# scomup/point-cloud-registration

Measured on AMD Instinct MI355X. Metric: M-correspondences/sec, plane calc_H_g_e2 on the B-01 stand-in (1.06 M pts), higher is better.
Workload: dtype f32; 1 GPU; plane_b01; kind=plane, target_points=1060000, scan_points_per_gpu=1060000, parallelism=scan-shard x1, devices_visible=1, scan_points_job=1060000, gauss_newton_iters_to_converge=5, correspondences_last_step=1060000

## Files before the change

### include/pcr.h

```cpp
#ifndef PCR_H
#define PCR_H

#include <stdint.h>

#ifdef __cplusplus
extern "C" {
#endif

#define PCR_API __attribute__((visibility("default")))

#define PCR_ABI_VERSION 5

typedef int pcr_status;
enum {
    PCR_OK = 0,
    PCR_ERR_INVALID = -1,
    PCR_ERR_HIP = -2,
    PCR_ERR_NO_TARGET = -3,
    PCR_ERR_COMM = -4,
    PCR_ERR_SINGULAR = -5,
    PCR_ERR_NOMEM = -6,
    PCR_ERR_UNSUPPORTED = -7
};

// ... 275 lines not shown
PCR_API pcr_status pcr_fgr_solo_max(pcr_context *ctx, int64_t *m_max);

#define PCR_COMPAT_M_MAX 32768
#define PCR_COMPAT_K_MAX 64
PCR_API pcr_status pcr_compat_bits(pcr_context *ctx, const float *src, const float *dst, int64_t m, double d,
                                   uint64_t *bits );
PCR_API pcr_status pcr_compat_degrees(pcr_context *ctx, const float *src, const float *dst, int64_t m, double d, int64_t *deg1 ,
                                      int64_t *deg2 );
PCR_API pcr_status pcr_compat_consensus(pcr_context *ctx, const float *src, const float *dst, int64_t m, double d, int n_seeds, int k,
                                        int64_t *deg1_or_null , int64_t *deg2_or_null , int32_t *seeds ,
                                        int32_t *members , int32_t *scores , int *n_seeds_out);

enum { PCR_K_LINEARIZE = 0, PCR_K_FINALIZE = 1, PCR_K_NN = 2, PCR_K_REDUCE = 3, PCR_K_ALLREDUCE = 4, PCR_K_CERTIFY = 5, PCR_K_COUNT = 6 };
PCR_API pcr_status pcr_profile_enable(pcr_context *ctx, int on);
PCR_API pcr_status pcr_profile_reset(pcr_context *ctx);
PCR_API pcr_status pcr_profile_read(pcr_context *ctx, int64_t launches[PCR_K_COUNT], double total_ms[PCR_K_COUNT]);
PCR_API pcr_status pcr_profile_read_n(pcr_context *ctx, int capacity, int64_t *launches, double *total_ms, int *count);
PCR_API pcr_status pcr_target_index_info(pcr_target *t, double *cell, int64_t dims[3], int64_t *occupied, int64_t *n);
PCR_API pcr_status pcr_target_index_population(pcr_target *t, int64_t *pop_max, int64_t *pop_p99, int *heavy);
PCR_API pcr_status pcr_target_index_x_order(pcr_target *t, double *xq);
PCR_API int pcr_x_order_rule(int f32_point_target, int heavy, int64_t n, int cell_bits);
PCR_API pcr_status pcr_target_index_halo(pcr_target *t, double *halo, int64_t *records);
PCR_API pcr_status pcr_target_index_halo2(pcr_target *t, double *halo, int64_t *records);
PCR_API pcr_status pcr_target_filter_band(pcr_target *t, double *band);
PCR_API pcr_status pcr_nn_counters(pcr_target *t, pcr_scan *s, const double T[16], double max_dist, double out[11]);
PCR_API pcr_status pcr_nn_counters_x(pcr_target *t, pcr_scan *s, const double T[16], double max_dist, double out[3]);
PCR_API pcr_status pcr_nn_counters_edge(pcr_target *t, pcr_scan *s, const double T[16], double max_dist, double out[9]);
PCR_API pcr_status pcr_set_variant(pcr_context *ctx, int variant);
PCR_API pcr_status pcr_get_variant(pcr_context *ctx, int *variant);
PCR_API pcr_status pcr_set_nn_mode(pcr_context *ctx, int mode);
PCR_API pcr_status pcr_set_reuse(pcr_context *ctx, int mode, double tau, double mu);
PCR_API pcr_status pcr_get_reuse(pcr_context *ctx, int *mode, double *tau, double *mu);
PCR_API pcr_status pcr_scan_reuse_stats(pcr_scan *s, double out[8]);
PCR_API pcr_status pcr_context_host_fold_passes(pcr_context *ctx, uint64_t *passes);
PCR_API pcr_status pcr_set_fuse_finalize(pcr_context *ctx, int on);
PCR_API int pcr_has_dev_kernels(void);
PCR_API pcr_status pcr_get_pipeline(pcr_context *ctx, int *variant, int *fuse_finalize, int *nn_mode);

#ifdef __cplusplus
}
#endif
#endif
```

### point_cloud_registration_amd/_capi.py

```python

import atexit
import ctypes as C
import os
import weakref

import numpy as np

_HERE = os.path.dirname(os.path.abspath(__file__))
LIB_PATH = os.environ.get("PCR_LIB") or os.path.join(_HERE, "libpcr_hip.so")
DEV_LIB_PATH = os.path.join(_HERE, "libpcr_hip_dev.so")

PCR_OK = 0
PCR_ERR_INVALID, PCR_ERR_HIP, PCR_ERR_NO_TARGET, PCR_ERR_COMM, PCR_ERR_SINGULAR, PCR_ERR_NOMEM = -1, -2, -3, -4, -5, -6
PCR_ERR_UNSUPPORTED = -7
ICP, PLANE, VPLANE, NDT = 0, 1, 2, 3
FLAG_ICP_RR_QUIRK = 1
FLAG_NO_SCAN_SORT = 2
FLAG_LOCAL_ONLY = 4
FLAG_HOST_LOOP = 8
FLAG_DEVICE_LOOP = 16
FLAG_KEEP_ORDER = 32
K_LINEARIZE, K_FINALIZE, K_NN, K_REDUCE, K_ALLREDUCE, K_CERTIFY, K_COUNT = 0, 1, 2, 3, 4, 5, 6
KERNEL_NAMES = ("linearize", "finalize", "nn", "reduce", "allreduce", "certify")
NN_FULL, NN_TRACK, NN_LIST = 0, 1, 2
# ... 80 lines not shown
    "pcr_profile_enable": (C.c_int, [_vp, C.c_int]),
    "pcr_profile_reset": (C.c_int, [_vp]),
    "pcr_profile_read": (C.c_int, [_vp, _i64p, _f64p]),
    "pcr_target_index_info": (C.c_int, [_vp, C.POINTER(C.c_double), _i64p, C.POINTER(C.c_int64), C.POINTER(C.c_int64)]),
    "pcr_target_index_halo": (C.c_int, [_vp, C.POINTER(C.c_double), C.POINTER(C.c_int64)]),
    "pcr_target_index_population": (C.c_int, [_vp, C.POINTER(C.c_int64), C.POINTER(C.c_int64), C.POINTER(C.c_int)]),
    "pcr_target_index_x_order": (C.c_int, [_vp, C.POINTER(C.c_double)]),
    "pcr_x_order_rule": (C.c_int, [C.c_int, C.c_int, C.c_int64, C.c_int]),
    "pcr_set_variant": (C.c_int, [_vp, C.c_int]),
    "pcr_get_variant": (C.c_int, [_vp, C.POINTER(C.c_int)]),
    "pcr_set_nn_mode": (C.c_int, [_vp, C.c_int]),
    "pcr_set_fuse_finalize": (C.c_int, [_vp, C.c_int]),
    "pcr_get_pipeline": (C.c_int, [_vp, C.POINTER(C.c_int), C.POINTER(C.c_int), C.POINTER(C.c_int)]),
    "pcr_nn_counters": (C.c_int, [_vp, _vp, _f64p, C.c_double, _f64p]),
    "pcr_nn_counters_x": (C.c_int, [_vp, _vp, _f64p, C.c_double, _f64p]),
    "pcr_nn_counters_edge": (C.c_int, [_vp, _vp, _f64p, C.c_double, _f64p]),
    "pcr_set_reuse": (C.c_int, [_vp, C.c_int, C.c_double, C.c_double]),
    "pcr_get_reuse": (C.c_int, [_vp, C.POINTER(C.c_int), C.POINTER(C.c_double), C.POINTER(C.c_double)]),
    "pcr_scan_reuse_stats": (C.c_int, [_vp, _f64p]),
    "pcr_context_host_fold_passes": (C.c_int, [_vp, C.POINTER(C.c_uint64)]),
    "pcr_hash64": (C.c_int, [_vp, C.c_uint64, C.POINTER(C.c_uint64)]),
    "pcr_target_filter_band": (C.c_int, [_vp, C.POINTER(C.c_double)]),
    "pcr_target_index_halo2": (C.c_int, [_vp, C.POINTER(C.c_double), C.POINTER(C.c_int64)]),
    "pcr_usable_cpus": (C.c_int, []),
    "pcr_has_dev_kernels": (C.c_int, []),
    "pcr_abi_version": (C.c_int, []),
    "pcr_context_trim": (C.c_int, [_vp, C.POINTER(C.c_uint64)]),
    "pcr_profile_read_n": (C.c_int, [_vp, C.c_int, _i64p, _f64p, C.POINTER(C.c_int)]),
    "pcr_scan_read_matches": (C.c_int, [_vp, _vp]),
    "pcr_comm_p2p_finegrained": (C.c_int, [_vp, C.POINTER(C.c_int)]),
    "pcr_lzf_decompress": (C.c_int, [_vp, C.c_uint64, _vp, C.c_uint64, C.POINTER(C.c_uint64)]),
    "pcr_lzf_compress": (C.c_int, [_vp, C.c_uint64, _vp, C.c_uint64, C.POINTER(C.c_uint64)]),
    "pcr_gn_set": (C.c_int, [_vp, _vp, C.c_int, _vp, C.c_int, C.c_int64, C.c_int, _f64p]),
    "pcr_coreset": (C.c_int, [_vp, _f64p, C.c_int, C.c_int64, _f64p, C.c_int, C.c_int64, C.POINTER(C.c_int64), _f64p, _i64p,
                              _f64p]),
    "pcr_linearize_rows": (C.c_int, [_vp, _vp, C.c_int, _f64p, C.c_double, C.c_uint, _vp, _vp, _vp, _vp, _vp]),
    "pcr_linearize_weighted": (C.c_int, [_vp, _vp, C.c_int, _f64p, C.c_double, C.c_uint, _f64p, _f64p]),
    "pcr_scan_coreset": (C.c_int, [_vp, _vp, C.c_int, _f64p, C.c_double, C.c_uint, C.c_int, C.c_int64, _i64p, _f64p,
                                   C.POINTER(C.c_int64)]),
    "pcr_target_estimate_covariances": (C.c_int, [_vp, C.c_int, C.c_int, C.c_double, _vp]),
    "pcr_target_set_covariances": (C.c_int, [_vp, _f32p]),
    "pcr_target_get_covariances": (C.c_int, [_vp, _f32p]),
    "pcr_scan_estimate_covariances": (C.c_int, [_vp, C.c_int, C.c_int, C.c_double, _vp]),
    "pcr_scan_set_covariances": (C.c_int, [_vp, _f32p]),
    "pcr_scan_get_covariances": (C.c_int, [_vp, _f32p]),
    "pcr_gicp_linearize": (C.c_int, [_vp, _vp, _f64p, C.c_double, C.c_uint, _f64p]),
# ... 508 lines not shown
        out = np.empty((self.size(), 6), np.float64)
        check(lib().pcr_target_voxels_get_covariances(self.handle, out))
        return out

    def voxel_stats(self, names=("mean", "cov", "norm", "icov", "counts", "keys")):
        n = self.size()
        bufs = {"mean": np.empty((n, 3)), "cov": np.empty((n, 3, 3)), "norm": np.empty((n, 3)),
                "icov": np.empty((n, 3, 3)), "counts": np.empty(n, np.int64), "keys": np.empty(n, np.int64)}
        nv = C.c_int64(0)
        args = [_ptr(bufs[k]) if k in names else None for k in ("mean", "cov", "norm", "icov", "counts", "keys")]
        check(lib().pcr_target_voxels_get(self.handle, C.byref(nv), *args))
        return {k: bufs[k] for k in names}

    def index_info(self):
        cell, occ, n = C.c_double(0), C.c_int64(0), C.c_int64(0)
        dims = np.zeros(3, np.int64)
        check(lib().pcr_target_index_info(self.handle, C.byref(cell), dims, C.byref(occ), C.byref(n)))
        halo, nh = C.c_double(0), C.c_int64(0)
        check(lib().pcr_target_index_halo(self.handle, C.byref(halo), C.byref(nh)))
        band = C.c_double(0)
        check(lib().pcr_target_filter_band(self.handle, C.byref(band)))
        halo2, nh2 = C.c_double(0), C.c_int64(0)
        check(lib().pcr_target_index_halo2(self.handle, C.byref(halo2), C.byref(nh2)))
        pmax, p99, heavy = C.c_int64(0), C.c_int64(0), C.c_int(0)
        check(lib().pcr_target_index_population(self.handle, C.byref(pmax), C.byref(p99), C.byref(heavy)))
        xq = C.c_double(0)
        check(lib().pcr_target_index_x_order(self.handle, C.byref(xq)))
        return {"cell": cell.value, "dims": tuple(int(d) for d in dims), "occupied": occ.value, "n": n.value,
                "halo": halo.value, "halo_records": nh.value, "filter_band": band.value,
                "halo2": halo2.value, "halo2_records": nh2.value,
                "pop_max": pmax.value, "pop_p99": p99.value, "heavy": bool(heavy.value),
                "x_ordered": xq.value > 0.0, "xq": xq.value}

    def searches_f64(self):
        return bool(self.is_voxel or getattr(self, "has_f64", False))

    def nn_query(self, q, r_max=np.inf):
        q = np.asarray(q)
        if q.dtype == np.float64 and self.searches_f64():
            q = np.ascontiguousarray(q)
            m = q.shape[0]
            dist, idx = np.empty(m, np.float64), np.empty(m, np.int64)
            check(lib().pcr_nn_query_dd(self.handle, q, m, float(r_max), dist, idx))
            return dist, idx
        q = np.ascontiguousarray(q, dtype=np.float32)
        m = q.shape[0]
        idx = np.empty(m, np.int64)
        if self.searches_f64():
            dist = np.empty(m, np.float64)
            check(lib().pcr_nn_query_f64(self.handle, q, m, float(r_max), dist, idx))
        else:
            dist = np.empty(m, np.float32)
            check(lib().pcr_nn_query(self.handle, q, m, float(r_max), dist, idx))
# ... 907 lines not shown
```

### point_cloud_registration_amd/csrc/api.hip

```cpp
#include <math.h>
#include <stdarg.h>
#include <stdlib.h>
#include <string.h>

#include <string>

#include "gn_math.h"
#include "pcr_internal.h"

static thread_local std::string g_last_error;

void pcr_set_error(const char *fmt, ...) {
    char buf[1024];
    va_list ap;
    va_start(ap, fmt);
    vsnprintf(buf, sizeof buf, fmt, ap);
    va_end(ap);
    g_last_error = buf;
}

extern "C" const char *pcr_last_error(void) { return g_last_error.c_str(); }
extern "C" const char *pcr_version(void) { return "pcr-hip 0.4 (gfx950)"; }
extern "C" int pcr_abi_version(void) { return PCR_ABI_VERSION; }

// ... 407 lines not shown
extern "C" pcr_status pcr_profile_read(pcr_context *ctx, int64_t launches[PCR_K_COUNT], double total_ms[PCR_K_COUNT]) {
    return pcr_profile_read_n(ctx, PCR_K_COUNT, launches, total_ms, nullptr);
}

template <typename T>
static pcr_status upload(pcr_context *ctx, const T *host, size_t count, DevBuf<T> *buf, bool exact = false, bool sync = true) {
    HIP_TRY(exact ? buf->alloc_exact(count) : buf->alloc(count));
    if (count) {
        HIP_TRY(hipMemcpyAsync(buf->p, host, sizeof(T) * count, hipMemcpyHostToDevice, ctx->stream));
        if (sync) HIP_TRY(hipStreamSynchronize(ctx->stream));
    }
    return PCR_OK;
}
static pcr_status synced(pcr_context *ctx, pcr_status s) {
    if (s != PCR_OK) (void)hipStreamSynchronize(ctx->stream);
    return s;
}

void pcr_target_release(pcr_target *t);
static void target_free(pcr_target *t) { pcr_target_release(t); }
void pcr_target_release(pcr_target *t) {
    if (!t) return;
    target_free(t->filter);
    void *ptrs[] = {t->cell_start, t->cell_seed, t->rowocc, t->lbox, t->gbox, t->lbox_h, t->gbox_h, t->lbox_h2, t->gbox_h2, t->cs_h, t->pts_h, t->j_h, t->cs_h2, t->pts_h2, t->j_h2, t->pts, t->pn, t->col, t->cint, t->gcov, t->pts64, t->means, t->vnorm, t->vicov, t->vcov,
                    t->st_mean, t->st_cov, t->st_norm, t->st_icov, t->st_counts, t->st_keys};
    if (t->ctx) (void)hipSetDevice(t->ctx->device);
    for (void *p : ptrs) pcr_persist_free(t->ctx, p);
    delete t;
}

static pcr_status points_create_common(pcr_context *ctx, const float *d_xyz, int64_t n, const float *d_normals,
                                       float cell_hint, pcr_target **out) {
    pcr_target *t = new pcr_target();
    t->ctx = ctx; t->is_voxel = 0; t->n = n; t->serial = ctx->next_serial++;
    pcr_status s = pcr_build_point_grid(ctx, d_xyz, n, cell_hint, t);
    if (s == PCR_OK && d_normals) {
        hipError_t e = pcr_persist_alloc((void **)&t->pn, sizeof(PtN) * (size_t)(n ? n : 1));
        if (e != hipSuccess) { pcr_set_error("hipMalloc normals: %s", hipGetErrorString(e)); s = PCR_ERR_HIP; }
        else s = pcr_permute_normals(ctx, d_normals, n, t->pts, t->pn);
        if (s == PCR_OK && hipStreamSynchronize(ctx->stream) != hipSuccess) s = PCR_ERR_HIP;
    }
    if (s != PCR_OK) { target_free(t); return s; }
    *out = t;
    return PCR_OK;
}

extern "C" pcr_status pcr_target_points_create(pcr_context *ctx, const float *xyz, int64_t n,
                                               const float *normals_or_null, float cell_hint, pcr_target **out) {
    PCR_REQUIRE(ctx && out, "NULL argument");
    PCR_REQUIRE(n >= 0 && (xyz || n == 0), "bad point array");
// ... 153 lines not shown
extern "C" pcr_status pcr_target_index_population(pcr_target *t, int64_t *pop_max, int64_t *pop_p99, int *heavy) {
    PCR_REQUIRE(t, "NULL argument");
    if (pop_max || pop_p99) {
        HIP_TRY(hipSetDevice(t->ctx->device));
        CtxScope scope(t->ctx);
        PCR_TRY(pcr_cell_population(t->ctx, t));
    }
    if (pop_max) *pop_max = t->pop_max;
    if (pop_p99) *pop_p99 = t->pop_p99;
    if (heavy) *heavy = t->heavy ? 1 : 0;
    return PCR_OK;
}

extern "C" pcr_status pcr_target_index_halo(pcr_target *t, double *halo, int64_t *records) {
    PCR_REQUIRE(t, "NULL argument");
    const pcr_target *p = t->is_voxel ? t->filter : t;
    if (halo) *halo = p ? (double)p->gf.halo : 0.0;
    if (records) *records = p ? p->n_h : 0;
    return PCR_OK;
}

extern "C" pcr_status pcr_target_index_halo2(pcr_target *t, double *halo, int64_t *records) {
    PCR_REQUIRE(t, "NULL argument");
    if (halo) *halo = t->is_voxel ? 0.0 : (double)t->halo2;
    if (records) *records = t->is_voxel ? 0 : t->n_h2;
    return PCR_OK;
}

extern "C" pcr_status pcr_target_filter_band(pcr_target *t, double *band) {
    PCR_REQUIRE(t && band, "NULL argument");
    *band = (t->is_voxel && t->filter) ? t->filter_band : 0.0;
    return PCR_OK;
}

extern "C" pcr_status pcr_target_destroy(pcr_target *t) {
    if (!t) return PCR_OK;
    (void)hipSetDevice(t->ctx->device);
    (void)hipStreamSynchronize(t->ctx->stream);
    target_free(t);
    return PCR_OK;
}

extern "C" pcr_status pcr_scan_create_device(pcr_context *ctx, const float *d_xyz, int64_t n, unsigned flags,
                                             pcr_scan **out) {
    PCR_REQUIRE(ctx && out, "NULL argument");
    PCR_REQUIRE(n >= 0 && (d_xyz || n == 0), "bad scan array");
    CtxScope scope(ctx);
    pcr_scan *s = new pcr_scan();
// ... 277 lines not shown
```

### point_cloud_registration_amd/csrc/index_build.hip

```cpp
#include <hipcub/hipcub.hpp>
#include <rocprim/rocprim.hpp>

#include <math.h>
#include <cmath>
#include <vector>

#include "nn_device.h"
#include "gn_math.h"

__device__ __forceinline__ unsigned f2ord(float f) {
    const unsigned u = __float_as_uint(f);
    return (u & 0x80000000u) ? ~u : (u | 0x80000000u);
}
static inline float ord2f(unsigned u) {
    const unsigned v = (u & 0x80000000u) ? (u & 0x7fffffffu) : ~u;
    float f;
    memcpy(&f, &v, 4);
    return f;
}

#define BBOX_SLOTS 64
#define BBOX_STRIDE 32
#define BBOX_WORDS (BBOX_STRIDE * (1 + BBOX_SLOTS))
template <typename T>
// ... 817 lines not shown
    const char *env = use_env ? getenv("PCR_GRID_CELL") : nullptr;
    bool auto_h = !(cell_hint > 0);
    if (env && atof(env) > 0) { h = atof(env); auto_h = false; }
    double halo = n <= ((int64_t)1 << 24) ? halo_default : 0.0;
    const char *he = getenv("PCR_HALO");
    if (he && *he) halo = atof(he);
    bool heavy = false;
    PCR_TRY((build_grid<float, float, PtF>(ctx, d_xyz, n, h, auto_h, &t->gf, &t->cell_start, &t->cell_seed, &t->pts, &t->occupied,
                                           halo, &t->cs_h, &t->pts_h, &t->j_h, &t->n_h, use_env ? &heavy : nullptr)));
    t->heavy = heavy;
    if (heavy) {
        PCR_TRY(make_leaf_boxes(ctx, t->pts, n, t->gf.h, t->gf.slack, &t->lbox, &t->gbox));
        t->gf.lbox = t->lbox; t->gf.gbox = t->gbox;
        if (t->pts_h) {
            PCR_TRY(make_leaf_boxes(ctx, t->pts_h, t->n_h, t->gf.h, t->gf.slack, &t->lbox_h, &t->gbox_h));
            t->gf.lbox_h = t->lbox_h; t->gf.gbox_h = t->gbox_h;
        }
        HIP_TRY(hipStreamSynchronize(ctx->stream));
    }
    return PCR_OK;
}

pcr_status pcr_build_deep_lists(pcr_context *ctx, pcr_target *t) {
    if (t->is_voxel || !t->cs_h || t->n <= 0 || t->cs_h2) return PCR_OK;
    {
        const char *de = getenv("PCR_DEEP_LISTS");
        if (de && atoi(de) == 0) return PCR_OK;
        size_t free_b = 0, total_b = 0;
        if (hipMemGetInfo(&free_b, &total_b) != hipSuccess) { (void)hipGetLastError(); free_b = 0; }
        const char *mb = getenv("PCR_DEEP_LISTS_MB");
        const double budget = mb && *mb ? atof(mb) * 1048576.0 : (double)free_b / 16.0;
        const double grow = (1.0 + 2.0 * PCR_HALO2_FRAC) * (1.0 + 2.0 * PCR_HALO2_FRAC) / (1.2 * 1.2);
        const double est = (double)(t->n_h > 0 ? t->n_h : t->n) * grow * 20.0 + 4.0 * ((double)t->gf.nx * t->gf.ny * t->gf.nz);
        if (est > budget) return PCR_OK;
    }
    DevBuf<uint32_t> cs_h, j_h;
    DevBuf<PtF> pts_h;
    int64_t n_h = 0;
    PCR_TRY(build_halo_lists(ctx, t->gf, t->pts, t->n, t->cell_start, PCR_HALO2_FRAC, &cs_h, &pts_h, &j_h, &n_h));
    if (n_h <= 0) return PCR_OK;
    t->halo2 = (float)(PCR_HALO2_FRAC * (double)t->gf.h);
    t->n_h2 = n_h;
    t->cs_h2 = cs_h.release(); t->pts_h2 = pts_h.release(); t->j_h2 = j_h.release();
    if (t->heavy) {
        PCR_TRY(make_leaf_boxes(ctx, t->pts_h2, n_h, t->gf.h, t->gf.slack, &t->lbox_h2, &t->gbox_h2));
        HIP_TRY(hipStreamSynchronize(ctx->stream));
    }
    return PCR_OK;
}

pcr_status pcr_build_centroid_grid(pcr_context *ctx, const double *d_mean, int64_t n, double cell, pcr_target *t) {
    uint32_t *cs_h = nullptr, *j_h = nullptr; PtF *pts_h = nullptr; int64_t n_h = 0;
    PCR_TRY((build_grid<double, double, PtD>(ctx, d_mean, n, cell, false, &t->gd, &t->cell_start, &t->cell_seed, &t->means, &t->occupied,
                                             0.0, &cs_h, &pts_h, &j_h, &n_h)));
    const char *oe = getenv("PCR_ROW_OCC");
    if (n > 0 && !(oe && atoi(oe) == 0)) PCR_TRY(make_row_occ<double>(ctx, t->cell_start, &t->gd, &t->rowocc));
    return PCR_OK;
}

__global__ void __launch_bounds__(256) k_means_to_f32(const PtD *__restrict__ means, int64_t n, float *__restrict__ xyz) {
    const int64_t j = (int64_t)blockIdx.x * 256 + threadIdx.x;
    if (j >= n) return;
    const PtD m = means[j];
    xyz[3 * j] = (float)m.x; xyz[3 * j + 1] = (float)m.y; xyz[3 * j + 2] = (float)m.z;
}

pcr_status pcr_build_centroid_filter(pcr_context *ctx, pcr_target *t) {
    if (t->n <= 0 || !ctx->vox_filter) return PCR_OK;
    const Geom<double> &g = t->gd;
// ... 211 lines not shown
```

### point_cloud_registration_amd/csrc/kernels.hip

```cpp
#include <type_traits>

#include "pass_device.h"
#ifdef PCR_DEV
#include "nn_mfma.h"
#endif

template <int VOXEL>
__global__ void __launch_bounds__(256) k_certify(const LinArgs a) {
    PoseK P;
    PoseQ Q;
    if (!load_pose<false>(a, P)) return;
    load_prev(a, Q);
    const TileIter it(a);
    const int lane = threadIdx.x & 63;
    uint32_t marked = 0;
    for (int64_t i0 = it.base - threadIdx.x; i0 < it.end; i0 += it.stride) {
        const int64_t i = i0 + threadIdx.x;
        const bool live = i < it.end;
        bool cert = false;
        if (live) {
            const uint32_t j = a.nn_j[i];
            const float lb = a.lb2[i];
            const float x = a.sx[i], y = a.sy[i], z = a.sz[i];
            float tx, ty, tz, ux, uy, uz;
// ... 151 lines not shown
__global__ void __launch_bounds__(256) k_nn_fix(const LinArgs a) {
    PoseK P;
    if (!load_pose<false>(a, P)) return;
    if (__builtin_amdgcn_readfirstlane(*(volatile const uint32_t *)a.pending) != a.stamp) return;
    for (int64_t i = (int64_t)blockIdx.x * 256 + threadIdx.x; i < a.n; i += (int64_t)gridDim.x * 256) {
        const uint32_t j = a.nn_j[i];
        if (nn_is_pending(j)) nn_point_fix(a, P, i, j & ~PCR_PENDING_BIT);
    }
}
#endif

__device__ __forceinline__ void pose_write(PoseDev *p, const double *T) {
    for (int i = 0; i < 16; ++i) p->T[i] = T[i];
    for (int i = 0; i < 3; ++i) {
        for (int j = 0; j < 3; ++j) { p->R[3 * i + j] = T[4 * i + j]; p->r32[3 * i + j] = (float)T[4 * i + j]; }
        p->t32[i] = (float)T[4 * i + 3];
    }
}
__device__ __forceinline__ void pose_arm(PoseDev *p, const double *T, int max_iter) {
    pose_write(p, T);
    p->iter = 0;
    p->done = max_iter > 0 ? PCR_LOOP_RUNNING : PCR_LOOP_MAXITER;
    p->tile_local = 0;
    p->halo_deep = 1;
}

__device__ __forceinline__ void gn_update(const FinArgs &f, double (*A)[7]) {
    PoseDev *p = f.pose;
    const int it = p->iter;
    double T[16];
    for (int i = 0; i < 16; ++i) T[i] = p->T[i];
    if (f.trace) {
        double *row = f.trace + (size_t)it * 45;
        for (int i = 0; i < 16; ++i) row[i] = T[i];
        for (int i = 0; i < 29; ++i) row[16 + i] = f.out[i];
    }
    double T_old[16];
    for (int i = 0; i < 16; ++i) T_old[i] = T[i];
    const int r = gn_step(A, f.out, f.tol, T);
    const double moved = r == 0 ? gn_typical_motion(T_old, T, f.bb_c, f.bb_e) : 0.0;
    p->tile_local = (r == 0 && f.local_len > 0.0 && moved < f.local_len) ? 1 : 0;
    p->halo_deep = (r == 0 && moved >= f.deep_len) ? 1 : 0;
    int done = r == 2 ? PCR_LOOP_SINGULAR : (r == 1 ? PCR_LOOP_CONVERGED : PCR_LOOP_RUNNING);
    if (r == 0) pose_write(p, T);
    const int it1 = it + 1;
    if (done == PCR_LOOP_RUNNING && it1 >= f.max_iter) done = PCR_LOOP_MAXITER;
    p->iter = it1;
    p->done = done;
    if (f.host_T) {
        if (done != PCR_LOOP_RUNNING) {
            for (int i = 0; i < 16; ++i) f.host_T[i] = T[i];
            __threadfence_system();
        }
        *f.host_state = ((unsigned long long)(unsigned)done << 32) | (unsigned)it1;
    }
}

__global__ void __launch_bounds__(64) k_gn_update(const FinArgs f) {
    if (threadIdx.x != 0) return;
    if (f.pose->done == PCR_LOOP_RUNNING) {
        double A[6][7];
        gn_update(f, A);
    } else if (f.pose->done == PCR_LOOP_COMMFAIL && f.host_state) {
        *f.host_state = ((unsigned long long)(unsigned)PCR_LOOP_COMMFAIL << 32) | (unsigned)f.pose->iter;
    }
// ... 331 lines not shown
```

### point_cloud_registration_amd/csrc/pass.hip

```cpp
#include <stdlib.h>

#include "pass_device.h"

static int grid8(int64_t want, int64_t cap = INT64_MAX) {
    int64_t nb = (want + 7) & ~(int64_t)7;
    if (nb > (cap & ~(int64_t)7)) nb = cap & ~(int64_t)7;
    return nb < 8 ? 8 : (int)nb;
}

#define PCR_HOST_ROWS_BYTES (sizeof(double) * 8 * 32 + sizeof(uint32_t) * 8 * PCR_GFLAG_STRIDE)

static double cell_edge(const pcr_target *t) { return t->is_voxel ? t->gd.h : (double)t->gf.h; }

pcr_status pcr_ensure_scratch(pcr_context *ctx, int64_t n_points) {
    (void)n_points;
    if (!ctx->d_partials) {
        ctx->max_blocks = (ctx->num_cu * 16 + 7) & ~7;
        HIP_TRY(pcr_malloc_retry((void **)&ctx->d_partials, sizeof(double) * 32 * (size_t)(ctx->max_blocks + 8)));
        HIP_TRY(pcr_malloc_retry((void **)&ctx->d_out, sizeof(double) * 32));
        HIP_TRY(pcr_malloc_retry((void **)&ctx->d_pose, sizeof(PoseDev)));
        HIP_TRY(hipHostMalloc(&ctx->h_out, sizeof(double) * 64, hipHostMallocMapped | hipHostMallocCoherent));
        memset(ctx->h_out, 0, sizeof(double) * 64);
        HIP_TRY(hipHostGetDevicePointer((void **)&ctx->h_out_dev, ctx->h_out, 0));
        HIP_TRY(hipHostMalloc((void **)&ctx->h_rows, PCR_HOST_ROWS_BYTES, hipHostMallocMapped | hipHostMallocCoherent));
// ... 12 lines not shown
        ctx->nn_blocks_per_cu[1] = blocks_per_cu(PCR_OCC_VOXEL, 4);
        ctx->nn_blocks_per_cu[3] = blocks_per_cu(PCR_OCC_FILTER, 4);
    }
    return PCR_OK;
}

static int64_t blocks_wanted(const pcr_context *ctx, int64_t n) {
    const int64_t want = (n + 255) / 256, cap = (int64_t)ctx->num_cu * 8;
    return want < cap ? want : cap;
}
int choose_blocks(const pcr_context *ctx, int64_t n) { return grid8(blocks_wanted(ctx, n), ctx->max_blocks); }

struct Pass {
    pcr_context *ctx;
    pcr_target *t;
    pcr_scan *s;
    int kind;
    LinArgs a;
    FinArgs f;
    bool one_kernel;
    bool fused_fin;
    bool gn_inline;
    double motion;
    int nn_mode;
    bool reuse_ready;
    bool q6;
};

bool pcr_pass_is_fused(const pcr_context *ctx, const pcr_scan *s) {
    if (ctx->variant == 2) return s->n <= (int64_t)ctx->num_cu * 1024;
    return ctx->variant == 0;
}

static void set_filter_bound(LinArgs &a, double bound);
#define PCR_PUBLIC_FLAGS (PCR_FLAG_ICP_RR_QUIRK | PCR_FLAG_NO_SCAN_SORT | PCR_FLAG_LOCAL_ONLY | PCR_FLAG_HOST_LOOP | PCR_FLAG_DEVICE_LOOP | PCR_FLAG_KEEP_ORDER)

static bool pass_is_q6(const pcr_target *t, int kind) { return kind == PCR_PLANE && !t->is_voxel && t->pts64 != nullptr; }

static pcr_status refuse_comm_and_q6(const pcr_target *t, int kind, const char *passes, const char *plane_passes, const char *q6_note) {
    if (t->ctx->comm != nullptr) pcr_set_error("%s are not available on a context with a communicator attached (pcr_comm_*, pcr_group)", passes);
    else if (pass_is_q6(t, kind)) pcr_set_error("%s are not available over a float64 point target (%s)", plane_passes, q6_note);
    else return PCR_OK;
    return PCR_ERR_UNSUPPORTED;
}

static void pass_init(Pass *ps, pcr_target *t, pcr_scan *s, int kind, bool one_kernel, bool q6) {
// ... 79 lines not shown
    if (pcr_build_deep_lists(ctx, t) != PCR_OK) (void)hipGetLastError();
}

static void pass_fill_lin(Pass *ps, double max_dist, unsigned flags, bool use_filter, bool deep, int nblocks) {
    const pcr_context *ctx = ps->ctx;
    const pcr_target *t = ps->t;
    const pcr_scan *s = ps->s;
    LinArgs &a = ps->a;
    memset(&a, 0, sizeof a);
    a.sx = s->x; a.sy = s->y; a.sz = s->z; a.n = s->n;
    a.gf = t->gf; a.pts = t->pts; a.pn = t->pn;
    a.pts_last = (uint32_t)(t->is_voxel ? 0 : t->n + PCR_PTS_PAD - 1);
    a.gd = t->gd; a.means = t->means; a.vnorm = t->vnorm; a.vicov = t->vicov;
    a.cell_start = t->cell_start;
    if (use_filter) {
        a.gf = t->filter->gf; a.pts = t->filter->pts; a.cs_f = t->filter->cell_start;
        a.band_f = (float)(t->filter_band * 1.000001);
    }
    if (ps->q6) {
        a.gd = t->gq; a.means = t->pts64; a.cs_f = t->cell_start;
        a.band_f = (float)(t->band64 * 1.000001);
        flags |= PCR_IFLAG_NOGATE;
    }
    if (deep && t->cs_h2) { a.cs_h2 = t->cs_h2; a.pts_h2 = t->pts_h2; a.j_h2 = t->j_h2; a.halo2_f = t->halo2; a.lbox_h2 = t->lbox_h2; a.gbox_h2 = t->gbox_h2; }
    a.md_f = (float)max_dist; a.md_d = max_dist;
    const double bound = max_dist * (1.0 + 1e-6);
    a.bound2_f = (float)(bound * bound); a.bound2_d = bound * bound;
    set_filter_bound(a, bound);
    a.flags = flags;
    a.nblocks = nblocks;
    a.partials = ctx->d_partials;
    a.nn_j = s->nn_j; a.tile_ctr = ctx->d_tile_ctr + 9 * PCR_TICKET_STRIDE;
    a.pending = ctx->d_tile_ctr + 9 * PCR_TICKET_STRIDE + (size_t)PCR_TILE_CTRS * PCR_TILE_STRIDE;
    a.lb2 = s->lb2; a.umask = s->umask; a.ucnt = s->ucnt;
    a.mu_f = (float)(ctx->reuse_mu * cell_edge(t));
}

static void pass_fill_fin(Pass *ps) {
    const pcr_context *ctx = ps->ctx;
    const pcr_scan *s = ps->s;
    FinArgs &f = ps->f;
    memset(&f, 0, sizeof f);
    for (int i = 0; i < 3; ++i) { f.bb_c[i] = s->bb_c[i]; f.bb_e[i] = s->bb_e[i]; }
    f.local_len = ctx->local_frac * cell_edge(ps->t);
    f.deep_len = PCR_HALO2_MOVE * cell_edge(ps->t);
    f.ucnt = s->ucnt; f.n_ucnt = ps->a.nblocks;
    f.partials = ctx->d_partials; f.tile_ctr = ctx->d_tile_ctr + 9 * PCR_TICKET_STRIDE; f.tickets = ctx->d_tile_ctr;
    f.nblocks = ps->a.nblocks; f.kind = ps->kind; f.out = ctx->d_out;
}

static pcr_status pass_setup(Pass *ps, pcr_target *t, pcr_scan *s, int kind, double max_dist, unsigned flags, bool force_fused = false) {
    pcr_context *ctx = t->ctx;
    PCR_TRY(pass_validate(t, s, kind, max_dist));
    HIP_TRY(hipSetDevice(ctx->device));
    PCR_TRY(pcr_ensure_scratch(ctx, s->n));
    const bool q6 = pass_is_q6(t, kind);
    const bool one_kernel = (force_fused || pcr_pass_is_fused(ctx, s)) && !q6;
    pass_init(ps, t, s, kind, one_kernel, q6);
    const int nblocks_split = grid8(choose_blocks(ctx, s->n), ctx->num_cu * 4);
    PCR_TRY(pass_scan_buffers(ps, nblocks_split));
    const bool filter_ok = t->is_voxel && ctx->vox_filter && ctx->nn_mode != 3 && (!one_kernel || ctx->fuse_finalize);
    if (filter_ok) pass_lazy_filter(ctx, t, one_kernel);
    const bool deep_ok = !t->is_voxel && !one_kernel && !q6 && t->cs_h && nn_plain(ctx);
    if (deep_ok) pass_lazy_deep_lists(ctx, t);
    pass_fill_lin(ps, max_dist, flags & PCR_PUBLIC_FLAGS, filter_ok && t->filter, deep_ok, one_kernel ? choose_blocks(ctx, s->n) : nblocks_split);
    pass_fill_fin(ps);
    return PCR_OK;
}
// ... 112 lines not shown
            else if (a.pose != nullptr) local = mode == PCR_NN_FULL ? 2 : 0;
            else if (ps->motion >= 0.0 && ps->motion < ps->f.local_len) local = 1;
        }
        if (ctx->tile_local >= 0) local = ctx->tile_local;
        ps->a.sched_local = local;
#ifdef PCR_DEV
        const bool mfma = !vox && !ps->q6 && mode == PCR_NN_FULL && ps->t->n > 0 && ctx->nn_mode == 4;
        if (coop) {
            pcr_dev_launch_coop(nn_grid, ctx->stream, a);
        } else if (mfma) {
            const int64_t nbm = (int64_t)ctx->num_cu * ctx->nn_blocks_per_cu[4];
            launch_nn_mfma(ps->t->cs_h != nullptr, ps->a.sched_local == 1 ? 1 : 0, dim3((unsigned)grid8(nbm < g.need ? nbm : g.need)), ctx->stream, a);
        } else
#endif
        if (filter) {
            if (++ctx->filter_stamp == 0) {
                HIP_TRY(hipMemsetAsync(a.pending, 0, 4, ctx->stream));
                ctx->filter_stamp = 1;
            }
            ps->a.stamp = ctx->filter_stamp;
            const bool fhalo = ps->q6 ? ps->t->cs_h != nullptr : ps->t->filter->cs_h != nullptr;
            launch_nn_filter(fhalo, ps->a.sched_local == 1 ? 1 : 0, !ps->fused_fin, ps->q6, nn_grid, ctx->stream, a);
        } else {
            if (!vox && a.pose == nullptr && a.halo2_f > 0.f && mode == PCR_NN_FULL && !(ps->motion >= 0.0 && ps->motion < ps->f.deep_len)) {
                ps->a.gf.halo = a.halo2_f; ps->a.gf.cs_h = a.cs_h2; ps->a.gf.pts_h = a.pts_h2; ps->a.gf.j_h = a.j_h2;
                ps->a.gf.lbox_h = a.lbox_h2; ps->a.gf.gbox_h = a.gbox_h2;
            }
            launch_plain_search(ps, nn_grid);
        }
        ps->s->nn_serial = ps->t->serial;
    }
    pcr_prof_end(ctx, &ev);
    return PCR_OK;
}

static void enqueue_reduce(Pass *ps, dim3 grid, bool filter) {
    pcr_context *ctx = ps->ctx;
    ProfEvent ev;
    pcr_prof_begin(ctx, PCR_K_REDUCE, &ev);
    RoctxRange range("pcr:reduce");
#ifdef PCR_DEV
    if (!ps->fused_fin) pcr_dev_launch_reduce(ps->kind, grid, ctx->stream, ps->a);
    else
#endif
    launch_reduce_kind(ps->kind, filter, grid, ctx->stream, ps->a, ps->f);
    pcr_prof_end(ctx, &ev);
}

static pcr_status pass_enqueue(Pass *ps) {
// ... 505 lines not shown
```

### point_cloud_registration_amd/csrc/pass_device.h

```cpp
#pragma once

#include <string.h>
#include <time.h>

#include <type_traits>

#include "gn_math.h"
#include "nn_device.h"

struct PoseK {
    float r32[9], t32[3];
    double R[9];
};
struct PoseQ {
    float r32[9], t32[3];
};

struct LinArgs {
    const float *sx, *sy, *sz;
    int64_t n;
    Geom<float> gf;
    const PtF *pts;
    uint32_t pts_last;
    const PtN *pn;
// ... 5 lines not shown
    PoseK hp;
    const PoseDev *pose;
    PoseQ hq;
    float *lb2;
    unsigned long long *umask;
    uint32_t *ucnt;
    float mu_f;
    float md_f;
    double md_d;
    float bound2_f;
    double bound2_d;
    const uint32_t *cs_f;
    float band_f;
    float mu_ff;
    float bound2_ff;
    uint32_t *pending;
    uint32_t stamp;
    unsigned flags;
    int nblocks;
    double *partials;
    uint32_t *nn_j;
    uint32_t *tile_ctr;
    int sched_local;
    const uint32_t *cs_h2;
    const void *pts_h2;
    const uint32_t *j_h2;
    float halo2_f;
    const float4 *lbox_h2, *gbox_h2;
};

struct RowArgs {
    const uint32_t *order;
    double *J, *r, *w, *W;
    int64_t *idx;
    uint32_t *flag, *inv;
    const uint32_t *off;
    double *P;
    int64_t stride;
    int64_t *col_idx;
};

__device__ __forceinline__ Geom<float> select_lists(const LinArgs &a) {
    Geom<float> g = a.gf;
    if (a.pose != nullptr && a.halo2_f > 0.f && __builtin_amdgcn_readfirstlane(a.pose->halo_deep) != 0) {
        g.halo = a.halo2_f; g.cs_h = a.cs_h2; g.pts_h = a.pts_h2; g.j_h = a.j_h2; g.lbox_h = a.lbox_h2; g.gbox_h = a.gbox_h2;
    }
    return g;
}

__device__ __forceinline__ float uniform_f32(float v) { return __int_as_float(__builtin_amdgcn_readfirstlane(__float_as_int(v))); }
__device__ __forceinline__ double uniform_f64(double v) {
    return __hiloint2double(__builtin_amdgcn_readfirstlane(__double2hiint(v)), __builtin_amdgcn_readfirstlane(__double2loint(v)));
}

template <bool NEED_R>
__device__ __forceinline__ bool load_pose(const LinArgs &a, PoseK &P) {
    if (a.pose == nullptr) { P = a.hp; return true; }
    const PoseDev *p = a.pose;
    if (__builtin_amdgcn_readfirstlane(p->done) != 0) return false;
#pragma unroll
    for (int i = 0; i < 9; ++i) P.r32[i] = uniform_f32(p->r32[i]);
#pragma unroll
    for (int i = 0; i < 3; ++i) P.t32[i] = uniform_f32(p->t32[i]);
    if (NEED_R) {
#pragma unroll
        for (int i = 0; i < 9; ++i) P.R[i] = uniform_f64(p->R[i]);
    }
    return true;
}
// ... 671 lines not shown
    uint32_t bj, bo;
    nn_box_f64(a.gd, a.means, a.cell_start, (double)tx, (double)ty, (double)tz, nominee, bd, bj, bo);
    a.nn_j[i] = __builtin_sqrt(bd) < a.md_d ? bj : PCR_NONE;
}

struct FinArgs {
    const double *partials;
    uint32_t *tile_ctr;
    uint32_t *tickets;
    int nblocks;
    int kind;
    double R[9];
    double *out;
    double *host_out;
    volatile uint32_t *host_flag;
    uint32_t seq;
    double *host_rows;
    volatile uint32_t *host_gflags;
    int nn_mode;
    const uint32_t *ucnt;
    int n_ucnt;
    float bb_c[3], bb_e[3];
    double local_len;
    double deep_len;
    PoseDev *pose;
    int max_iter;
    double tol;
    double *trace;
    double *host_T;
    volatile unsigned long long *host_state;
};

struct BatchItem {
    const float *sx, *sy, *sz;
    int64_t n;
    double *partials;
    uint32_t *tickets;
    PoseDev *pose;
    double *out;
    double *trace;
    double *host_T;
    unsigned long long *host_state;
    int nblocks;
    int pad;
    float bb_c[3], bb_e[3];
    double T[16];
};
// ... 176 lines not shown
```

### point_cloud_registration_amd/csrc/pcr_internal.h

```cpp
#pragma once

#include <hip/hip_runtime.h>
#include <stdint.h>
#include <stdio.h>
#include <mutex>
#include <unordered_map>
#include <utility>
#include <vector>

#include "pcr.h"

void pcr_set_error(const char *fmt, ...);

#define HIP_TRY(expr)                                                                          \
    do {                                                                                       \
        hipError_t e_ = (expr);                                                                \
        if (e_ != hipSuccess) {                                                                \
            pcr_set_error("%s failed: %s (%s:%d)", #expr, hipGetErrorString(e_), __FILE__, __LINE__); \
            return PCR_ERR_HIP;                                                                \
        }                                                                                      \
    } while (0)

#define PCR_TRY(expr)                      \
    do {                                   \
// ... 21 lines not shown
    Real slack;
    int nx, ny, nz;
    uint32_t cs_mask;
    const uint32_t *seed;
    Real halo;
    const uint32_t *cs_h;
    const void *pts_h;
    const uint32_t *j_h;
    const unsigned long long *rowocc;
    int nyw, nxb;
    const float4 *lbox, *gbox, *lbox_h, *gbox_h;
    Real xq;
    [[no_unique_address]] GeomSwitches<Real> sw;
};
static_assert(sizeof(Geom<float>) == 136 && sizeof(Geom<double>) == 160, "Geom is a kernel argument: its layout is pinned");
#define PCR_LB_MIN 24
#ifndef PCR_HALO2_FRAC
#define PCR_HALO2_FRAC 0.25
#endif
#define PCR_HALO2_AFTER 12
#ifndef PCR_HALO2_MOVE
#define PCR_HALO2_MOVE 0.12
#endif
#define PCR_GAP_SHIFT 28
#define PCR_GAP_MAX 15

typedef float4 PtF;
typedef double4 PtD;
struct __attribute__((aligned(32))) PtN {
    float x, y, z;
    uint32_t orig;
    float nx, ny, nz;
    uint32_t pad;
};

struct PoseDev {
    double T[16];
    double R[9];
    float r32[9], t32[3];
    int iter;
    int done;
    int tile_local;
    int halo_deep;
};
#define PCR_LOOP_RUNNING 0
#define PCR_LOOP_CONVERGED 1
// ... 116 lines not shown
    bool prof_this_pass = false;
    std::vector<ProfEvent> prof_events;
    std::vector<ProfEvent> prof_free;
    int64_t prof_launches[PCR_K_COUNT] = {0};
    double prof_ms[PCR_K_COUNT] = {0};
    void *comm = nullptr;
    int comm_kind = 0;
    int nranks = 1, rank = 0;
    std::recursive_mutex cache_mu;
    size_t cache_limit = (size_t)1 << 30;
    std::vector<std::pair<size_t, void *>> cache;
    size_t cache_bytes = 0;
    std::unordered_map<void *, size_t> owned;
};

struct pcr_target {
    pcr_context *ctx = nullptr;
    int is_voxel = 0;
    int64_t n = 0;
    int64_t occupied = 0;
    uint32_t *cell_start = nullptr;
    uint32_t *cell_seed = nullptr;
    unsigned long long *rowocc = nullptr;
    float4 *lbox = nullptr, *gbox = nullptr, *lbox_h = nullptr, *gbox_h = nullptr, *lbox_h2 = nullptr, *gbox_h2 = nullptr;
    int64_t pop_max = 0, pop_p99 = 0;
    bool heavy = false;
    uint32_t *cs_h = nullptr;
    PtF *pts_h = nullptr;
    uint32_t *j_h = nullptr;
    int64_t n_h = 0;
    uint32_t *cs_h2 = nullptr;
    PtF *pts_h2 = nullptr;
    uint32_t *j_h2 = nullptr;
    int64_t n_h2 = 0;
    float halo2 = 0;
    int split_passes = 0;
    bool deep_tried = false;
    Geom<float> gf;
    PtF *pts = nullptr;
    PtN *pn = nullptr;
    float4 *col = nullptr;
    float *cint = nullptr;
    float *gcov = nullptr;
    uint64_t serial = 0;
    PtD *pts64 = nullptr;
    double band64 = 0;
    Geom<double> gq;
    Geom<double> gd;
    PtD *means = nullptr;
    double *vnorm = nullptr;
    double *vicov = nullptr;
    double *vcov = nullptr;
    double *st_mean = nullptr, *st_cov = nullptr, *st_norm = nullptr, *st_icov = nullptr;
    int64_t *st_counts = nullptr, *st_keys = nullptr;
    double voxel_size = 0;
    pcr_target *filter = nullptr;
    double filter_band = 0;
    int fused_passes = 0;
// ... 114 lines not shown
```

Measured before the change: 10880 Mcorr/s.

## Add a third, wider halo list set selected by pose motion

Generalizes the single deep halo list into an array of list sets, building a wider halo (0.35 cell) alongside the 0.25 one for non-heavy targets. The per-iteration device flag now selects among the base, medium and far list sets depending on how far the pose moved, and falls back to the base lists when motion is very large. The aim is to keep large-motion early Gauss-Newton iterations on precomputed halo lists, so the search avoids slower multi-cell neighbor visits. It costs extra memory and build time for the additional list set, and a wider halo means more points scanned per query.

```diff
diff --git a/include/pcr.h b/include/pcr.h
--- a/include/pcr.h
+++ b/include/pcr.h
@@ -321,6 +321,7 @@
 PCR_API int pcr_x_order_rule(int f32_point_target, int heavy, int64_t n, int cell_bits);
 PCR_API pcr_status pcr_target_index_halo(pcr_target *t, double *halo, int64_t *records);
 PCR_API pcr_status pcr_target_index_halo2(pcr_target *t, double *halo, int64_t *records);
+PCR_API pcr_status pcr_target_index_list_set(pcr_target *t, int set, double *halo, int64_t *records);
 PCR_API pcr_status pcr_target_filter_band(pcr_target *t, double *band);
 PCR_API pcr_status pcr_nn_counters(pcr_target *t, pcr_scan *s, const double T[16], double max_dist, double out[11]);
 PCR_API pcr_status pcr_nn_counters_x(pcr_target *t, pcr_scan *s, const double T[16], double max_dist, double out[3]);
diff --git a/point_cloud_registration_amd/_capi.py b/point_cloud_registration_amd/_capi.py
--- a/point_cloud_registration_amd/_capi.py
+++ b/point_cloud_registration_amd/_capi.py
@@ -126,6 +126,7 @@
     "pcr_hash64": (C.c_int, [_vp, C.c_uint64, C.POINTER(C.c_uint64)]),
     "pcr_target_filter_band": (C.c_int, [_vp, C.POINTER(C.c_double)]),
     "pcr_target_index_halo2": (C.c_int, [_vp, C.POINTER(C.c_double), C.POINTER(C.c_int64)]),
+    "pcr_target_index_list_set": (C.c_int, [_vp, C.c_int, C.POINTER(C.c_double), C.POINTER(C.c_int64)]),
     "pcr_usable_cpus": (C.c_int, []),
     "pcr_has_dev_kernels": (C.c_int, []),
     "pcr_abi_version": (C.c_int, []),
@@ -680,13 +681,18 @@
         check(lib().pcr_target_filter_band(self.handle, C.byref(band)))
         halo2, nh2 = C.c_double(0), C.c_int64(0)
         check(lib().pcr_target_index_halo2(self.handle, C.byref(halo2), C.byref(nh2)))
+        sets = []
+        for k in range(3):
+            hk, nk = C.c_double(0), C.c_int64(0)
+            check(lib().pcr_target_index_list_set(self.handle, k, C.byref(hk), C.byref(nk)))
+            sets.append((hk.value, nk.value))
         pmax, p99, heavy = C.c_int64(0), C.c_int64(0), C.c_int(0)
         check(lib().pcr_target_index_population(self.handle, C.byref(pmax), C.byref(p99), C.byref(heavy)))
         xq = C.c_double(0)
         check(lib().pcr_target_index_x_order(self.handle, C.byref(xq)))
         return {"cell": cell.value, "dims": tuple(int(d) for d in dims), "occupied": occ.value, "n": n.value,
                 "halo": halo.value, "halo_records": nh.value, "filter_band": band.value,
-                "halo2": halo2.value, "halo2_records": nh2.value,
+                "halo2": halo2.value, "halo2_records": nh2.value, "list_sets": sets,
                 "pop_max": pmax.value, "pop_p99": p99.value, "heavy": bool(heavy.value),
                 "x_ordered": xq.value > 0.0, "xq": xq.value}
 
diff --git a/point_cloud_registration_amd/csrc/api.hip b/point_cloud_registration_amd/csrc/api.hip
--- a/point_cloud_registration_amd/csrc/api.hip
+++ b/point_cloud_registration_amd/csrc/api.hip
@@ -453,10 +453,12 @@
 void pcr_target_release(pcr_target *t) {
     if (!t) return;
     target_free(t->filter);
-    void *ptrs[] = {t->cell_start, t->cell_seed, t->rowocc, t->lbox, t->gbox, t->lbox_h, t->gbox_h, t->lbox_h2, t->gbox_h2, t->cs_h, t->pts_h, t->j_h, t->cs_h2, t->pts_h2, t->j_h2, t->pts, t->pn, t->col, t->cint, t->gcov, t->pts64, t->means, t->vnorm, t->vicov, t->vcov,
+    void *ptrs[] = {t->cell_start, t->cell_seed, t->rowocc, t->lbox, t->gbox, t->lbox_h, t->gbox_h, t->cs_h, t->pts_h, t->j_h, t->pts, t->pn, t->col, t->cint, t->gcov, t->pts64, t->means, t->vnorm, t->vicov, t->vcov,
                     t->st_mean, t->st_cov, t->st_norm, t->st_icov, t->st_counts, t->st_keys};
     if (t->ctx) (void)hipSetDevice(t->ctx->device);
     for (void *p : ptrs) pcr_persist_free(t->ctx, p);
+    for (const pcr_target::ListSet &d : t->deep)
+        for (void *p : {(void *)d.cs, (void *)d.pts, (void *)d.j, (void *)d.lbox, (void *)d.gbox}) pcr_persist_free(t->ctx, p);
     delete t;
 }
 
@@ -656,8 +658,16 @@
 
 extern "C" pcr_status pcr_target_index_halo2(pcr_target *t, double *halo, int64_t *records) {
     PCR_REQUIRE(t, "NULL argument");
-    if (halo) *halo = t->is_voxel ? 0.0 : (double)t->halo2;
-    if (records) *records = t->is_voxel ? 0 : t->n_h2;
+    if (halo) *halo = t->is_voxel ? 0.0 : (double)t->deep[0].halo;
+    if (records) *records = t->is_voxel ? 0 : t->deep[0].n;
+    return PCR_OK;
+}
+
+extern "C" pcr_status pcr_target_index_list_set(pcr_target *t, int set, double *halo, int64_t *records) {
+    PCR_REQUIRE(t && set >= 0 && set <= PCR_DEEP_SETS, "NULL argument or no such list set");
+    if (set == 0) return pcr_target_index_halo(t, halo, records);
+    if (halo) *halo = t->is_voxel ? 0.0 : (double)t->deep[set - 1].halo;
+    if (records) *records = t->is_voxel ? 0 : t->deep[set - 1].n;
     return PCR_OK;
 }
 
diff --git a/point_cloud_registration_amd/csrc/index_build.hip b/point_cloud_registration_amd/csrc/index_build.hip
--- a/point_cloud_registration_amd/csrc/index_build.hip
+++ b/point_cloud_registration_amd/csrc/index_build.hip
@@ -863,29 +863,32 @@
 }
 
 pcr_status pcr_build_deep_lists(pcr_context *ctx, pcr_target *t) {
-    if (t->is_voxel || !t->cs_h || t->n <= 0 || t->cs_h2) return PCR_OK;
-    {
-        const char *de = getenv("PCR_DEEP_LISTS");
-        if (de && atoi(de) == 0) return PCR_OK;
-        size_t free_b = 0, total_b = 0;
-        if (hipMemGetInfo(&free_b, &total_b) != hipSuccess) { (void)hipGetLastError(); free_b = 0; }
-        const char *mb = getenv("PCR_DEEP_LISTS_MB");
-        const double budget = mb && *mb ? atof(mb) * 1048576.0 : (double)free_b / 16.0;
-        const double grow = (1.0 + 2.0 * PCR_HALO2_FRAC) * (1.0 + 2.0 * PCR_HALO2_FRAC) / (1.2 * 1.2);
-        const double est = (double)(t->n_h > 0 ? t->n_h : t->n) * grow * 20.0 + 4.0 * ((double)t->gf.nx * t->gf.ny * t->gf.nz);
-        if (est > budget) return PCR_OK;
-    }
-    DevBuf<uint32_t> cs_h, j_h;
-    DevBuf<PtF> pts_h;
-    int64_t n_h = 0;
-    PCR_TRY(build_halo_lists(ctx, t->gf, t->pts, t->n, t->cell_start, PCR_HALO2_FRAC, &cs_h, &pts_h, &j_h, &n_h));
-    if (n_h <= 0) return PCR_OK;
-    t->halo2 = (float)(PCR_HALO2_FRAC * (double)t->gf.h);
-    t->n_h2 = n_h;
-    t->cs_h2 = cs_h.release(); t->pts_h2 = pts_h.release(); t->j_h2 = j_h.release();
-    if (t->heavy) {
-        PCR_TRY(make_leaf_boxes(ctx, t->pts_h2, n_h, t->gf.h, t->gf.slack, &t->lbox_h2, &t->gbox_h2));
-        HIP_TRY(hipStreamSynchronize(ctx->stream));
+    if (t->is_voxel || !t->cs_h || t->n <= 0 || t->deep[0].cs) return PCR_OK;
+    const char *de = getenv("PCR_DEEP_LISTS");
+    if (de && atoi(de) == 0) return PCR_OK;
+    size_t free_b = 0, total_b = 0;
+    if (hipMemGetInfo(&free_b, &total_b) != hipSuccess) { (void)hipGetLastError(); free_b = 0; }
+    const char *mb = getenv("PCR_DEEP_LISTS_MB");
+    const double budget = mb && *mb ? atof(mb) * 1048576.0 : (double)free_b / 16.0;
+    const double frac[PCR_DEEP_SETS] = {PCR_HALO2_FRAC, PCR_HALO3_FRAC};
+    double used = 0.0;
+    for (int k = 0; k < (t->heavy ? 1 : PCR_DEEP_SETS); ++k) {
+        const double grow = (1.0 + 2.0 * frac[k]) * (1.0 + 2.0 * frac[k]) / (1.2 * 1.2);
+        used += (double)(t->n_h > 0 ? t->n_h : t->n) * grow * 20.0 + 4.0 * ((double)t->gf.nx * t->gf.ny * t->gf.nz);
+        if (used > budget) break;
+        DevBuf<uint32_t> cs_h, j_h;
+        DevBuf<PtF> pts_h;
+        int64_t n_h = 0;
+        PCR_TRY(build_halo_lists(ctx, t->gf, t->pts, t->n, t->cell_start, frac[k], &cs_h, &pts_h, &j_h, &n_h));
+        if (n_h <= 0) break;
+        pcr_target::ListSet &d = t->deep[k];
+        d.halo = (float)(frac[k] * (double)t->gf.h);
+        d.n = n_h;
+        d.cs = cs_h.release(); d.pts = pts_h.release(); d.j = j_h.release();
+        if (t->heavy) {
+            PCR_TRY(make_leaf_boxes(ctx, d.pts, n_h, t->gf.h, t->gf.slack, &d.lbox, &d.gbox));
+            HIP_TRY(hipStreamSynchronize(ctx->stream));
+        }
     }
     return PCR_OK;
 }
diff --git a/point_cloud_registration_amd/csrc/kernels.hip b/point_cloud_registration_amd/csrc/kernels.hip
--- a/point_cloud_registration_amd/csrc/kernels.hip
+++ b/point_cloud_registration_amd/csrc/kernels.hip
@@ -197,7 +197,7 @@
     p->iter = 0;
     p->done = max_iter > 0 ? PCR_LOOP_RUNNING : PCR_LOOP_MAXITER;
     p->tile_local = 0;
-    p->halo_deep = 1;
+    p->halo_deep = PCR_DEEP_SETS;
 }
 
 __device__ __forceinline__ void gn_update(const FinArgs &f, double (*A)[7]) {
@@ -215,7 +215,7 @@
     const int r = gn_step(A, f.out, f.tol, T);
     const double moved = r == 0 ? gn_typical_motion(T_old, T, f.bb_c, f.bb_e) : 0.0;
     p->tile_local = (r == 0 && f.local_len > 0.0 && moved < f.local_len) ? 1 : 0;
-    p->halo_deep = (r == 0 && moved >= f.deep_len) ? 1 : 0;
+    p->halo_deep = (r != 0 || moved >= f.out_len) ? 0 : (moved >= f.far_len ? 2 : (moved >= f.deep_len ? 1 : 0));
     int done = r == 2 ? PCR_LOOP_SINGULAR : (r == 1 ? PCR_LOOP_CONVERGED : PCR_LOOP_RUNNING);
     if (r == 0) pose_write(p, T);
     const int it1 = it + 1;
diff --git a/point_cloud_registration_amd/csrc/pass.hip b/point_cloud_registration_amd/csrc/pass.hip
--- a/point_cloud_registration_amd/csrc/pass.hip
+++ b/point_cloud_registration_amd/csrc/pass.hip
@@ -58,6 +58,7 @@
     bool fused_fin;
     bool gn_inline;
     double motion;
+    bool list_force;
     int nn_mode;
     bool reuse_ready;
     bool q6;
@@ -183,7 +184,18 @@
         a.band_f = (float)(t->band64 * 1.000001);
         flags |= PCR_IFLAG_NOGATE;
     }
-    if (deep && t->cs_h2) { a.cs_h2 = t->cs_h2; a.pts_h2 = t->pts_h2; a.j_h2 = t->j_h2; a.halo2_f = t->halo2; a.lbox_h2 = t->lbox_h2; a.gbox_h2 = t->gbox_h2; }
+    if (deep) {
+        const char *fe = getenv("PCR_LIST_SET");
+        const int force = fe && *fe ? atoi(fe) : -1;
+        for (int k = 0, have = -1; k < PCR_DEEP_SETS; ++k) {
+            if (t->deep[k].cs) have = k;
+            const int use = force < 0 ? have : (force >= 1 && force <= PCR_DEEP_SETS && t->deep[force - 1].cs ? force - 1 : -1);
+            if (use < 0) continue;
+            const pcr_target::ListSet &d = t->deep[use];
+            a.deep[k].cs = d.cs; a.deep[k].pts = d.pts; a.deep[k].j = d.j; a.deep[k].lbox = d.lbox; a.deep[k].gbox = d.gbox; a.deep[k].halo = d.halo;
+        }
+        ps->list_force = force >= 1 && a.deep[0].halo > 0.f;
+    }
     a.md_f = (float)max_dist; a.md_d = max_dist;
     const double bound = max_dist * (1.0 + 1e-6);
     a.bound2_f = (float)(bound * bound); a.bound2_d = bound * bound;
@@ -205,6 +217,9 @@
     for (int i = 0; i < 3; ++i) { f.bb_c[i] = s->bb_c[i]; f.bb_e[i] = s->bb_e[i]; }
     f.local_len = ctx->local_frac * cell_edge(ps->t);
     f.deep_len = PCR_HALO2_MOVE * cell_edge(ps->t);
+    f.far_len = PCR_HALO3_MOVE * cell_edge(ps->t);
+    f.out_len = ps->t->heavy ? HUGE_VAL : PCR_HALO_OUT_MOVE * cell_edge(ps->t);
+    if (ps->list_force) { f.deep_len = f.far_len = 0.0; f.out_len = HUGE_VAL; }
     f.ucnt = s->ucnt; f.n_ucnt = ps->a.nblocks;
     f.partials = ctx->d_partials; f.tile_ctr = ctx->d_tile_ctr + 9 * PCR_TICKET_STRIDE; f.tickets = ctx->d_tile_ctr;
     f.nblocks = ps->a.nblocks; f.kind = ps->kind; f.out = ctx->d_out;
@@ -363,9 +378,10 @@
             const bool fhalo = ps->q6 ? ps->t->cs_h != nullptr : ps->t->filter->cs_h != nullptr;
             launch_nn_filter(fhalo, ps->a.sched_local == 1 ? 1 : 0, !ps->fused_fin, ps->q6, nn_grid, ctx->stream, a);
         } else {
-            if (!vox && a.pose == nullptr && a.halo2_f > 0.f && mode == PCR_NN_FULL && !(ps->motion >= 0.0 && ps->motion < ps->f.deep_len)) {
-                ps->a.gf.halo = a.halo2_f; ps->a.gf.cs_h = a.cs_h2; ps->a.gf.pts_h = a.pts_h2; ps->a.gf.j_h = a.j_h2;
-                ps->a.gf.lbox_h = a.lbox_h2; ps->a.gf.gbox_h = a.gbox_h2;
+            if (!vox && a.pose == nullptr && mode == PCR_NN_FULL) {
+                const double m = ps->motion;
+                const int k = m < 0.0 ? 1 : (m >= ps->f.out_len ? -1 : (m >= ps->f.far_len ? 1 : (m >= ps->f.deep_len ? 0 : -1)));
+                if (k >= 0 && a.deep[k].halo > 0.f) use_lists(ps->a.gf, a.deep[k]);
             }
             launch_plain_search(ps, nn_grid);
         }
diff --git a/point_cloud_registration_amd/csrc/pass_device.h b/point_cloud_registration_amd/csrc/pass_device.h
--- a/point_cloud_registration_amd/csrc/pass_device.h
+++ b/point_cloud_registration_amd/csrc/pass_device.h
@@ -51,11 +51,13 @@
     uint32_t *nn_j;
     uint32_t *tile_ctr;
     int sched_local;
-    const uint32_t *cs_h2;
-    const void *pts_h2;
-    const uint32_t *j_h2;
-    float halo2_f;
-    const float4 *lbox_h2, *gbox_h2;
+    struct DeepLists {
+        const uint32_t *cs;
+        const void *pts;
+        const uint32_t *j;
+        const float4 *lbox, *gbox;
+        float halo;
+    } deep[PCR_DEEP_SETS];
 };
 
 struct RowArgs {
@@ -69,11 +71,14 @@
     int64_t *col_idx;
 };
 
+__host__ __device__ __forceinline__ void use_lists(Geom<float> &g, const LinArgs::DeepLists &d) {
+    g.halo = d.halo; g.cs_h = d.cs; g.pts_h = d.pts; g.j_h = d.j; g.lbox_h = d.lbox; g.gbox_h = d.gbox;
+}
 __device__ __forceinline__ Geom<float> select_lists(const LinArgs &a) {
     Geom<float> g = a.gf;
-    if (a.pose != nullptr && a.halo2_f > 0.f && __builtin_amdgcn_readfirstlane(a.pose->halo_deep) != 0) {
-        g.halo = a.halo2_f; g.cs_h = a.cs_h2; g.pts_h = a.pts_h2; g.j_h = a.j_h2; g.lbox_h = a.lbox_h2; g.gbox_h = a.gbox_h2;
-    }
+    const int k = a.pose != nullptr ? __builtin_amdgcn_readfirstlane(a.pose->halo_deep) : 0;
+    if (k >= 2 && a.deep[1].halo > 0.f) use_lists(g, a.deep[1]);
+    else if (k >= 1 && a.deep[0].halo > 0.f) use_lists(g, a.deep[0]);
     return g;
 }
 
@@ -791,7 +796,8 @@
     int n_ucnt;
     float bb_c[3], bb_e[3];
     double local_len;
-    double deep_len;
+    double deep_len, far_len;
+    double out_len;
     PoseDev *pose;
     int max_iter;
     double tol;
diff --git a/point_cloud_registration_amd/csrc/pcr_internal.h b/point_cloud_registration_amd/csrc/pcr_internal.h
--- a/point_cloud_registration_amd/csrc/pcr_internal.h
+++ b/point_cloud_registration_amd/csrc/pcr_internal.h
@@ -67,6 +67,16 @@
 #ifndef PCR_HALO2_MOVE
 #define PCR_HALO2_MOVE 0.12
 #endif
+#ifndef PCR_HALO3_FRAC
+#define PCR_HALO3_FRAC 0.35
+#endif
+#ifndef PCR_HALO3_MOVE
+#define PCR_HALO3_MOVE 0.4
+#endif
+#ifndef PCR_HALO_OUT_MOVE
+#define PCR_HALO_OUT_MOVE 1.5
+#endif
+#define PCR_DEEP_SETS 2
 #define PCR_GAP_SHIFT 28
 #define PCR_GAP_MAX 15
 
@@ -229,18 +239,21 @@
     uint32_t *cell_start = nullptr;
     uint32_t *cell_seed = nullptr;
     unsigned long long *rowocc = nullptr;
-    float4 *lbox = nullptr, *gbox = nullptr, *lbox_h = nullptr, *gbox_h = nullptr, *lbox_h2 = nullptr, *gbox_h2 = nullptr;
+    float4 *lbox = nullptr, *gbox = nullptr, *lbox_h = nullptr, *gbox_h = nullptr;
     int64_t pop_max = 0, pop_p99 = 0;
     bool heavy = false;
     uint32_t *cs_h = nullptr;
     PtF *pts_h = nullptr;
     uint32_t *j_h = nullptr;
     int64_t n_h = 0;
-    uint32_t *cs_h2 = nullptr;
-    PtF *pts_h2 = nullptr;
-    uint32_t *j_h2 = nullptr;
-    int64_t n_h2 = 0;
-    float halo2 = 0;
+    struct ListSet {
+        uint32_t *cs = nullptr;
+        PtF *pts = nullptr;
+        uint32_t *j = nullptr;
+        float4 *lbox = nullptr, *gbox = nullptr;
+        int64_t n = 0;
+        float halo = 0;
+    } deep[PCR_DEEP_SETS];
     int split_passes = 0;
     bool deep_tried = false;
     Geom<float> gf;
```

New measurement: 11130 Mcorr/s, median of 6. 2.3% higher.
